# arangesh/TrackMPNN

Hardware: AMD Instinct MI355X
Metric: graph_edges_per_sec_fwd_bwd (higher is better)
Workload: dtype f32; 1 GPU; C2 KITTI Car/RRC-shaped rolling windows: 7 frames, D_t~clip(Poisson(6),1,20), F=8 (2d), H=64, K=0, diff; 1 fwd per frame + 1 bwd per window; 16384 windows/GPU batched block-diagonally (64 distinct seeds tiled); windows_per_gpu=16384, rows_final=6762496, parallelism=sequence-dp1

## Files before the change

include/tmpnn.h:

```cpp
#ifndef TMPNN_H
#define TMPNN_H

#include <stddef.h>
#include <stdint.h>

#ifdef __cplusplus
extern "C" {
#endif

#define TMPNN_ABI_VERSION 10

#define TMPNN_OK 0
#define TMPNN_EINVAL (-1)
#define TMPNN_ELAUNCH (-2)
#define TMPNN_EWORKSPACE (-3)

typedef void* tmpnn_stream;
typedef void* tmpnn_event;

typedef struct tmpnn_seg_plan {
    int32_t T;
    int32_t I;
    int32_t nsplit;
    const int32_t* t_row;
    const int32_t* items;
// ... 99 lines not shown
                          const float* dy, const float* w_head,
                          float* dW_ih, float* dW_hh, float* db_ih, float* db_hh,
                          void* ws, size_t ws_bytes, tmpnn_stream stream);

int tmpnn_gru_bwd_fused_available(int H, int IN, int xmode);
size_t tmpnn_gru_bwd_fused_ws(int R, int IN, int H);
int tmpnn_gru_bwd_fused(const int32_t* rows, int R, int xmode, const int32_t* src, const int32_t* dst,
                        const float* msg, int ld_msg, int msg_compact, int IN,
                        const float* h, int ld_h, int H, const float* w_ih, const float* w_hh,
                        const float* gates, size_t gate_plane, const float* d_hout, int ld_dhout,
                        const float* dy, const float* w_head,
                        float* d_msg, int ld_dmsg, float* d_h, int ld_dh,
                        const int32_t* add_src, const int32_t* add_dst, const float* add_msg, int ld_add,
                        float* dW_ih, float* dW_hh, float* db_ih, float* db_hh,
                        void* ws, size_t ws_bytes, tmpnn_stream stream);
typedef struct tmpnn_zs_gate_src {
    const float* proj;
    int32_t ld_proj;
    const int32_t* src_pos;
    const int32_t* dst_pos;
    const float* b_ih;
    const float* b_hh;
} tmpnn_zs_gate_src;
int tmpnn_gru_bwd_fused_zero_state_available(int H, int IN, int xmode);
int tmpnn_gru_bwd_fused_zero_state(const int32_t* rows, int R, const int32_t* src, const int32_t* dst, int IN,
                                   const float* h, int ld_h, int H, const float* w_ih, const float* b_hn,
                                   const float* gates, size_t gate_plane, const float* d_hout, int ld_dhout,
                                   const float* dy, const float* w_head, float* d_msg, int ld_dmsg,
                                   float* dW_ih, float* db_ih, float* db_hh,
                                   void* ws, size_t ws_bytes, tmpnn_stream stream);

int tmpnn_gru_fwd_tiles(const tmpnn_edge_tiles* tiles, int R, const float* proj, int ld_proj, const float* h, int ld_h, int H,
                        const float* whh_t, const float* b_ih, const float* b_hh, float* h_out, int ld_out, float* gates,
                        size_t gate_plane, const float* w_head, float* logit_part, size_t part_stride, tmpnn_stream stream);
int tmpnn_gru_fwd_tiles_zero_state_available(int H, int xmode);
int tmpnn_gru_fwd_tiles_zero_state(const tmpnn_edge_tiles* tiles, int R, const float* proj, int ld_proj, int H,
                                   const float* b_ih, const float* b_hh, float* h_out, int ld_out, float* gates,
// ... 373 lines not shown
```

trackmpnn_amd/_lib.py:

```python
from __future__ import annotations

import ctypes as C

import torch
import os
import re
from typing import Dict, List, Optional

_HERE = os.path.dirname(os.path.abspath(__file__))
LIB_PATH = os.environ.get('TMPNN_LIB_PATH') or os.path.join(_HERE, 'lib', 'libtmpnn.so')
HEADER_PATH = os.path.join(os.path.dirname(_HERE), 'include', 'tmpnn.h')

ABI_VERSION = 10

c_int = C.c_int
c_void_p = C.c_void_p
c_size_t = C.c_size_t
c_float = C.c_float


class CSegPlan(C.Structure):
    _fields_ = [('T', C.c_int32), ('I', C.c_int32), ('nsplit', C.c_int32), ('t_row', c_void_p), ('items', c_void_p),
                ('rowptr2', c_void_p), ('inc2', c_void_p), ('ws', c_void_p), ('ws_floats', c_size_t)]


class CWinPlan(C.Structure):
    _fields_ = [('W', C.c_int32), ('nbig', C.c_int32), ('wrec', c_void_p), ('erow', c_void_p), ('recs', c_void_p),
                ('det', c_void_p), ('drow', c_void_p), ('big_order', c_void_p)]


class CGraph(C.Structure):
    _fields_ = [('N', C.c_int32), ('E', C.c_int32), ('Dn', C.c_int32),
                ('src', c_void_p), ('dst', c_void_p), ('edge_row', c_void_p), ('det_row', c_void_p),
                ('rowptr', c_void_p), ('inc', c_void_p), ('det_order', c_void_p), ('seg_plan', c_void_p),
                ('win_plan', c_void_p)]


_GP = C.POINTER(CGraph)


class CZsGateSrc(C.Structure):
    _fields_ = [('proj', c_void_p), ('ld_proj', C.c_int32), ('src_pos', c_void_p), ('dst_pos', c_void_p),
                ('b_ih', c_void_p), ('b_hh', c_void_p)]


class CEdgeTiles(C.Structure):
    _fields_ = [('T', C.c_int32), ('rows_per_tile', C.c_int32), ('t_row', c_void_p), ('t_loc', c_void_p),
                ('t_dptr', c_void_p), ('t_dets', c_void_p)]


_TP = C.POINTER(CEdgeTiles)


class CDGraph(C.Structure):
    _fields_ = [('N', C.c_int32), ('cap', C.c_int32), ('meta', c_void_p), ('is_edge', c_void_p), ('pos', c_void_p),
                ('src', c_void_p), ('dst', c_void_p), ('src_pos', c_void_p), ('dst_pos', c_void_p),
                ('edge_row', c_void_p), ('det_row', c_void_p), ('rowptr', c_void_p), ('inc', c_void_p)]

# ... 296 lines not shown
```

trackmpnn_amd/csrc/gru_bwd.hip:

```cpp
#include "gru_common.h"

namespace tmpnn {



template <int NT>
__global__ __launch_bounds__(256) void k_gru_bwd_data(GruBwdDataArgs a) {
    const int wave = threadIdx.x >> 6, lane = threadIdx.x & 63;
    const int c = lane & 31, half = lane >> 5;
    const int r0 = (blockIdx.x * 4 + wave) * 32;
    if (r0 >= a.R) return;
    const int H = a.H;
    const int vcol0 = blockIdx.y * (32 * NT);
    const bool is_dx = vcol0 < a.IN;
    const int n0 = is_dx ? vcol0 : vcol0 - a.IN;
    const float* __restrict__ W = is_dx ? a.w_ih : a.w_hh;
    const int ldw = is_dx ? a.IN : H;
    const int li = min(r0 + c, a.R - 1);
    const int row = a.rows[li];
    const size_t gp = a.gate_plane;

    f32x16 acc[NT];
#pragma unroll
    for (int t = 0; t < NT; ++t)
// ... 1760 lines not shown
        for (int j = 0; j < 3; ++j) {
            const float tot = bsum[j] + __shfl_xor(bsum[j], 32);
            if (half == 0) red[wave * 96 + j * 32 + c32] = tot;
        }
        __syncthreads();
        if (HHS && tt == 0 && half == 0) {
            float* sb = a.slab_b + (size_t)blockIdx.x * 6 * H;
#pragma unroll
            for (int j = 0; j < 3; ++j)
                sb[role * 3 * H + (jt0 + j) * 32 + c32] = red[wave * 96 + j * 32 + c32] + red[(wave + 1) * 96 + j * 32 + c32];
        }
    }
}

struct ZsGateSrc { const float* proj; int ld_proj; const int32_t* src_pos; const int32_t* dst_pos; const float* b_ih; const float* b_hh; };

__device__ __forceinline__ float zs_gate(float ps, float pd, float bsum) { return sigmoidf_((0.0f + (ps - pd)) + bsum); }
__device__ __forceinline__ float zs_gate_n(float ps, float pd, float b_in, float r, float b_hn) {
    return tanhf_(gru_n_preact((ps - pd) + b_in, r, 0.0f + b_hn));
}

template <int UP, bool RC = false>
__global__ __launch_bounds__(512) void k_gru_bwd_zs(GruBwdFusedArgs a, const float* __restrict__ b_hn, int ntiles) {
    constexpr int H = 64;
    constexpr int SUB = 32 * 128;
    constexpr int PA = 2 * SUB, PB = SUB;
    constexpr int OFF_B = 3 * PA;
    constexpr int BUF = OFF_B + 3 * PB;
    extern __shared__ float lds[];
    uint16_t* const lds16 = reinterpret_cast<uint16_t*>(lds);
    const int tid = threadIdx.x;
    const int wave = __builtin_amdgcn_readfirstlane(tid >> 6), lane = tid & 63;
    const int role = wave >> 2, q = wave & 3;
    const int j16 = lane & 15, kq = lane >> 4;
    const int srow = 4 * wave + kq, f4 = 4 * j16;
    const int n0 = 16 * q;
    uint4 wq[6][3];
#pragma unroll
    for (int s6 = 0; s6 < 6; ++s6) {
        const int ch = s6 < 4 ? 4 * kq + s6 : 16 + 4 * (s6 - 4) + kq;
        float v[8];
#pragma unroll
        for (int i = 0; i < 8; ++i) v[i] = a.w_ih[(size_t)(8 * ch + i) * a.ld_wih + n0 + j16];
        const Split8 sp = split8_arr(v);
        wq[s6][0] = sp.p1; wq[s6][1] = sp.p2; wq[s6][2] = sp.p3;
    }
    const float headl = (UP & 2) ? a.up.w_head[lane] : 0.f;
    const float4 bhn = *reinterpret_cast<const float4*>(b_hn + f4);
    const int st0 = dui_off(srow, f4);
    const int swzj = dui_swz(j16), rowj = (16 * role + j16) * 128;
    const int half = lane >> 5, c32 = lane & 31;
    const int jt0 = (q >> 1) * 3, tt = q & 1;
    const int i16 = lane & 15, tq = i16 >> 2, tp = i16 & 3, tg = (lane >> 4) & 1;
    const int trow = (8 * half + tq) * 128, tsw0 = (tq << 2) | (2 * half);
    const int kofs = role * 2048;
    int offA[3], offB;
#pragma unroll
    for (int j = 0; j < 3; ++j) {
        const int col = (jt0 + j) * 32;
        const int ch = ((col & 127) >> 3) + 2 * tg + (tp >> 1);
        offA[j] = kofs + (col >> 7) * SUB + trow + ((ch ^ tsw0) << 3) + 4 * (tp & 1);
    }
    {
// ... 3 lines not shown
    f32x16 acc[3];
#pragma unroll
    for (int j = 0; j < 3; ++j)
#pragma unroll
        for (int i = 0; i < 16; ++i) acc[j][i] = 0.f;
    float bs_r[4] = {0.f, 0.f, 0.f, 0.f}, bs_z[4] = {0.f, 0.f, 0.f, 0.f};
    float bs_n[4] = {0.f, 0.f, 0.f, 0.f}, bs_nr[4] = {0.f, 0.f, 0.f, 0.f};

    const int G = gridDim.x;
    const int nmine = (ntiles - (int)blockIdx.x + G - 1) / G;
    struct { float4 dh, r, z, n, xa, xb; float dy; } raw;
    float d0[4], tv[4];
    struct { float4 pa, pb, qa, qb, na, nb; } rp;
    const ZsGateSrc gsrc{a.msg, a.ld_msg, a.add_src, a.add_dst, a.add_msg, b_hn - 2 * H};
    float* const sgb = lds + BUF;
    if constexpr (RC) {
        if (tid < 3 * H) sgb[tid] = tid < 2 * H ? gsrc.b_ih[tid] + gsrc.b_hh[tid] : gsrc.b_ih[tid];
        __syncthreads();
    }
    auto row_of = [&](int tile, bool tvld, bool& vld) -> int {
        const int lr = tile * 32 + srow;
        vld = tvld && lr < a.R;
        return vld ? lr : a.R - 1;
    };
#define ZS_SLICE(SL, img, vld)                                                                               \
    do {                                                                                                     \
        float o_[4];                                                                                         \
        if ((SL) == 0) {                                                                                     \
            const float dh_[4] = {raw.dh.x, raw.dh.y, raw.dh.z, raw.dh.w}, r_[4] = {raw.r.x, raw.r.y, raw.r.z, raw.r.w}; \
            const float z_[4] = {raw.z.x, raw.z.y, raw.z.z, raw.z.w}, n_[4] = {raw.n.x, raw.n.y, raw.n.z, raw.n.w}; \
            const float hn_[4] = {bhn.x, bhn.y, bhn.z, bhn.w};                                               \
            _Pragma("unroll") for (int i = 0; i < 4; ++i) {                                                  \
// ... 33 lines not shown
            raw.n = TWO_LD4(g0_ + 2 * gp_);                                                                  \
            raw.z = TWO_LD4(g0_ + gp_);                                                                      \
        }                                                                                                    \
    } while (0)
#define ZS_ISSUE_GATHER(gs_, gd_)                                                                            \
    do {                                                                                                     \
        raw.xa = *reinterpret_cast<const float4*>(a.h + (size_t)(gs_) * a.ld_h + f4);                        \
        raw.xb = *reinterpret_cast<const float4*>(a.h + (size_t)(gd_) * a.ld_h + f4);                        \
    } while (0)

#define ZS_ISSUE_P(G3, A_, B_, sp_, dp_)                                                                     \
    do {                                                                                                     \
        rp.A_ = *reinterpret_cast<const float4*>(gsrc.proj + (size_t)(sp_) * gsrc.ld_proj + (G3) * H + f4); \
        rp.B_ = *reinterpret_cast<const float4*>(gsrc.proj + (size_t)(dp_) * gsrc.ld_proj + (G3) * H + f4); \
    } while (0)
#define ZS_GATE(G3, A_, B_, OUT_)                                                                            \
    do {                                                                                                     \
        const float4 b_ = *reinterpret_cast<const float4*>(sgb + (G3) * H + f4);                             \
        raw.OUT_ = make_float4(zs_gate(rp.A_.x, rp.B_.x, b_.x), zs_gate(rp.A_.y, rp.B_.y, b_.y),             \
                               zs_gate(rp.A_.z, rp.B_.z, b_.z), zs_gate(rp.A_.w, rp.B_.w, b_.w));            \
    } while (0)
#define ZS_GATE_N()                                                                                          \
    do {                                                                                                     \
        const float4 b_ = *reinterpret_cast<const float4*>(sgb + 2 * H + f4);                                \
        raw.n = make_float4(zs_gate_n(rp.na.x, rp.nb.x, b_.x, raw.r.x, bhn.x),                               \
                            zs_gate_n(rp.na.y, rp.nb.y, b_.y, raw.r.y, bhn.y),                               \
                            zs_gate_n(rp.na.z, rp.nb.z, b_.z, raw.r.z, bhn.z),                               \
                            zs_gate_n(rp.na.w, rp.nb.w, b_.w, raw.r.w, bhn.w));                              \
    } while (0)
#define ZS_ISSUE_DH(orow_)                                                                                   \
// ... 8 lines not shown
    int sp_n = 0, dp_n = 0;
    if constexpr (RC) {
        bool v0, v1;
        const int lp0 = row_of(blockIdx.x, true, v0);
        const int o0 = a.rows[lp0];
        gs_cur = a.src[lp0]; gd_cur = a.dst[lp0];
        const int sp0 = gsrc.src_pos[lp0], dp0 = gsrc.dst_pos[lp0];
        ZS_ISSUE_DH(o0); ZS_ISSUE_GATHER(gs_cur, gd_cur);
        ZS_ISSUE_P(0, pa, pb, sp0, dp0); ZS_ISSUE_P(1, qa, qb, sp0, dp0); ZS_ISSUE_P(2, na, nb, sp0, dp0);
        const int lp1 = row_of(blockIdx.x + G, 1 < nmine, v1);
        const int o1 = a.rows[lp1];
        const int sp1 = gsrc.src_pos[lp1], dp1 = gsrc.dst_pos[lp1];
        ZS_GATE(0, pa, pb, r); ZS_GATE(1, qa, qb, z); ZS_GATE_N();
        ZS_SLICE(0, lds16, v0); ZS_SLICE(1, lds16, v0); ZS_SLICE(3, lds16, v0); ZS_SLICE(5, lds16, v0);
        ZS_ISSUE_DH(o1);
        ZS_ISSUE_P(0, pa, pb, sp1, dp1); ZS_GATE(0, pa, pb, r);
        ZS_ISSUE_P(1, qa, qb, sp1, dp1); ZS_GATE(1, qa, qb, z);
        ZS_ISSUE_P(2, na, nb, sp1, dp1); ZS_GATE_N();
        valid_cur = v1;
        gs_cur = a.src[lp1]; gd_cur = a.dst[lp1];
        const int lp2 = row_of(blockIdx.x + 2 * G, 2 < nmine, valid_n);
        orow_n = a.rows[lp2];
        sp_n = gsrc.src_pos[lp2]; dp_n = gsrc.dst_pos[lp2];
    } else {
        bool v0, v1;
        const int lp0 = row_of(blockIdx.x, true, v0);
        const int o0 = a.rows[lp0];
        gs_cur = a.src[lp0]; gd_cur = a.dst[lp0];
        ZS_ISSUE_MAIN(0, o0); ZS_ISSUE_MAIN(1, o0); ZS_ISSUE_GATHER(gs_cur, gd_cur);
        const int lp1 = row_of(blockIdx.x + G, 1 < nmine, v1);
        const int o1 = a.rows[lp1];
        ZS_SLICE(0, lds16, v0); ZS_ISSUE_MAIN(0, o1);
        ZS_SLICE(1, lds16, v0); ZS_ISSUE_MAIN(1, o1);
        ZS_SLICE(3, lds16, v0);
        ZS_SLICE(5, lds16, v0);
        valid_cur = v1;
        gs_cur = a.src[lp1]; gd_cur = a.dst[lp1];
        const int lp2 = row_of(blockIdx.x + 2 * G, 2 < nmine, valid_n);
        orow_n = a.rows[lp2];
    }
    __syncthreads();

    for (int it = 0; it < nmine; ++it) {
        const int tile = blockIdx.x + it * G;
        uint16_t* const cur = lds16 + (it & 1) * BUF;
        uint16_t* const nxt = lds16 + ((it & 1) ^ 1) * BUF;
        const int er = a.rows[min(tile * 32 + 16 * role + j16, a.R - 1)];
        const bool el = tile * 32 + 16 * role + j16 < a.R;
        f32x4 accd;
#pragma unroll
        for (int i = 0; i < 4; ++i) accd[i] = 0.f;
#pragma unroll
        for (int s6 = 0; s6 < 6; ++s6) {
            uint4 bd[3];
            const uint16_t* pd;
            {
                const int chunk = s6 < 4 ? 4 * kq + s6 : 4 * (s6 - 4) + kq;
                pd = cur + (s6 >= 4 ? SUB : 0) + rowj + ((chunk ^ swzj) << 3);
            }
            if (s6 < 3) {
                uint4 aw[3], bt[3];
                {
                    const uint16_t* p0 = cur + offB;
                    const uint16_t* p1 = cur + (offB ^ 8) + 4 * 128;
#pragma unroll
                    for (int pc = 0; pc < 3; ++pc) {
                        const uint2 u0 = lds_read_tr(p0 + pc * PB), u1 = lds_read_tr(p1 + pc * PB);
                        bt[pc] = make_uint4(u0.x, u0.y, u1.x, u1.y);
                    }
                }
                const uint16_t* p0 = cur + offA[s6];
                const uint16_t* p1 = cur + (offA[s6] ^ 8) + 4 * 128;
#pragma unroll
                for (int pc = 0; pc < 3; ++pc) {
                    const uint2 u0 = lds_read_tr(p0 + pc * PA), u1 = lds_read_tr(p1 + pc * PA);
                    aw[pc] = make_uint4(u0.x, u0.y, u1.x, u1.y);
                }
                if constexpr (RC) {
                    if (s6 == 0) {
                        ZS_SLICE(0, nxt, valid_cur); ZS_SLICE(1, nxt, valid_cur);
                        ZS_ISSUE_DH(orow_n);
                    } else if (s6 == 1) {
                        ZS_SLICE(3, nxt, valid_cur);
                        ZS_ISSUE_GATHER(gs_cur, gd_cur);
                    } else {
                        ZS_ISSUE_P(0, pa, pb, sp_n, dp_n);
                    }
                } else {
                    ZS_SLICE(s6, nxt, valid_cur);
                    ZS_ISSUE_MAIN(s6, orow_n);
                }
                acc[s6] = mfma32_c<0>(aw, bt, acc[s6]); acc[s6] = mfma32_c<1>(aw, bt, acc[s6]);
                acc[s6] = mfma32_c<2>(aw, bt, acc[s6]); acc[s6] = mfma32_c<3>(aw, bt, acc[s6]);
                acc[s6] = mfma32_c<4>(aw, bt, acc[s6]); acc[s6] = mfma32_c<5>(aw, bt, acc[s6]);
            } else if constexpr (RC) {
                if (s6 == 3) {
                    ZS_SLICE(5, nxt, valid_cur);
                    ZS_ISSUE_P(1, qa, qb, sp_n, dp_n);
                } else if (s6 == 4) {
                    ZS_ISSUE_P(2, na, nb, sp_n, dp_n);
                    ZS_GATE(0, pa, pb, r);
                } else {
                    ZS_GATE(1, qa, qb, z);
                    ZS_GATE_N();
                }
            } else {
                ZS_SLICE(s6, nxt, valid_cur);
                if (s6 == 3) ZS_ISSUE_GATHER(gs_cur, gd_cur);
            }
#pragma unroll
            for (int pc = 0; pc < 3; ++pc) bd[pc] = *reinterpret_cast<const uint4*>(pd + pc * PA);
            accd = mfma16_c<0>(wq[s6], bd, accd); accd = mfma16_c<1>(wq[s6], bd, accd);
            accd = mfma16_c<2>(wq[s6], bd, accd); accd = mfma16_c<3>(wq[s6], bd, accd);
            accd = mfma16_c<4>(wq[s6], bd, accd); accd = mfma16_c<5>(wq[s6], bd, accd);
            __builtin_amdgcn_sched_barrier(0);
        }
        {
            bool vnn;
            const int lp2 = row_of(tile + 2 * G, it + 2 < nmine, vnn);
            gs_cur = a.src[lp2]; gd_cur = a.dst[lp2];
            valid_cur = valid_n;
            const int lp3 = row_of(tile + 3 * G, it + 3 < nmine, valid_n);
            orow_n = a.rows[lp3];
            if constexpr (RC) { sp_n = gsrc.src_pos[lp3]; dp_n = gsrc.dst_pos[lp3]; }
            (void)vnn;
        }
        int cofs = n0 + 4 * kq;
        asm volatile("" : "+v"(cofs));
        if (el) *reinterpret_cast<float4*>(a.d_msg + ((size_t)er * a.ld_dmsg + cofs)) =
                    make_float4(accd[0], accd[1], accd[2], accd[3]);
        __syncthreads();
    }
#undef ZS_ISSUE_DH
#undef ZS_GATE_N
#undef ZS_GATE
#undef ZS_ISSUE_P
#undef ZS_ISSUE_GATHER
#undef ZS_ISSUE_MAIN
#undef ZS_SLICE
    float* sw = a.slab_w + (size_t)blockIdx.x * (3 * H) * (2 * H);
#pragma unroll
    for (int j = 0; j < 3; ++j)
#pragma unroll
        for (int reg = 0; reg < 16; ++reg) {
            const int jj = (jt0 + j) * 32 + acc_row(reg, half);
            sw[(size_t)jj * (2 * H) + role * H + tt * 32 + c32] = acc[j][reg];
        }
    {
        float* red = lds;
        *reinterpret_cast<float4*>(red + srow * 256 + 0 * 64 + f4) = make_float4(bs_r[0], bs_r[1], bs_r[2], bs_r[3]);
// ... 380 lines not shown
int tmpnn_gru_bwd_fused_zero_state_available(int H, int IN, int xmode) {
    return (H == 64 && IN == 64 && xmode == 1 && device_gives_160k()) ? 1 : 0;
}

int tmpnn_gru_bwd_fused_zero_state(const int32_t* rows, int R, const int32_t* src, const int32_t* dst, int IN,
                                   const float* h, int ld_h, int H, const float* w_ih, const float* b_hn,
                                   const float* gates, size_t gate_plane, const float* d_hout, int ld_dhout,
                                   const float* dy, const float* w_head, float* d_msg, int ld_dmsg, float* dW_ih,
                                   float* db_ih, float* db_hh, void* ws, size_t ws_bytes, tmpnn_stream stream) {
    TM_REQUIRE(tmpnn_gru_bwd_fused_zero_state_available(H, IN, 1), "gru_bwd_fused_zero_state: H=%d IN=%d not supported", H, IN);
    if (R == 0) return TMPNN_OK;
    TM_REQUIRE(R > 0 && rows && src && dst && h && w_ih && b_hn && gates && d_msg && dW_ih && db_ih && db_hh,
               "gru_bwd_fused_zero_state: null pointer");
    const bool rc_gates = gate_plane == 0;
    ZsGateSrc gsrc{};
    if (rc_gates) {
        const tmpnn_zs_gate_src* g = reinterpret_cast<const tmpnn_zs_gate_src*>(gates);
        TM_REQUIRE(g->proj && g->src_pos && g->dst_pos && g->b_ih && g->b_hh,
                   "gru_bwd_fused_zero_state: gate_plane = 0 needs proj, src_pos, dst_pos, b_ih and b_hh (struct tmpnn_zs_gate_src)");
        TM_REQUIRE(aligned16(g->proj) && g->ld_proj >= 3 * H && (g->ld_proj & 3) == 0 && aligned16(g->b_ih) && aligned16(g->b_hh),
                   "gru_bwd_fused_zero_state: gate source layout (16-byte alignment, ld_proj=%d)", (int)g->ld_proj);
        TM_REQUIRE(b_hn == g->b_hh + 2 * H, "gru_bwd_fused_zero_state: b_hn is not b_hh + 2H of the gate source");
        gsrc = ZsGateSrc{g->proj, g->ld_proj, g->src_pos, g->dst_pos, g->b_ih, g->b_hh};
        gates = nullptr;
    }
    TM_REQUIRE(d_hout != nullptr || dy != nullptr, "gru_bwd_fused_zero_state: no upstream gradient");
    TM_REQUIRE(dy == nullptr || (w_head != nullptr && aligned16(w_head)),
               "gru_bwd_fused_zero_state: dy needs a 16-byte aligned w_head");
    TM_REQUIRE((ld_h & 3) == 0 && aligned16(h) && aligned16(gates) && (gate_plane & 3) == 0 && aligned16(w_ih) &&
                   aligned16(b_hn) && (d_hout == nullptr || ((ld_dhout & 3) == 0 && aligned16(d_hout))) &&
                   (ld_dmsg & 3) == 0 && aligned16(d_msg) && ld_dmsg >= IN && ld_h >= H,
               "gru_bwd_fused_zero_state: rows must be 16-byte aligned");
    const size_t need = tmpnn_gru_bwd_fused_ws(R, IN, H);
    if (ws == nullptr || ws_bytes < need)
        return set_error(TMPNN_EWORKSPACE, "gru_bwd_fused_zero_state: workspace %zu < %zu bytes", ws_bytes, need);
    const int n_rs = fused_blocks(R);
    const size_t nW = (size_t)3 * H * (IN + H), nB = (size_t)6 * H;
    float* slab_w = reinterpret_cast<float*>(ws);
    float* slab_b = slab_w + (size_t)n_rs * nW;
    float* fold = slab_b + (size_t)n_rs * nB;
    GruBwdFusedArgs a{rows, R, src, dst, nullptr, 0, 0, h, ld_h, w_ih, nullptr, gates, gate_plane,
                      DhSrc{d_hout, ld_dhout, dy, w_head}, d_msg, ld_dmsg, nullptr, 0, nullptr, nullptr, nullptr, 0,
                      slab_w, slab_b, IN};
    if (rc_gates) {
        a.msg = gsrc.proj; a.ld_msg = gsrc.ld_proj;
        a.add_src = gsrc.src_pos; a.add_dst = gsrc.dst_pos; a.add_msg = gsrc.b_ih;
    }
    const int ntiles = ceil_div(R, 32);
    const size_t shm = 147456;
    hipStream_t st = as_stream(stream);
    const int up = (d_hout ? 1 : 0) | (dy ? 2 : 0);
#define LZ(U)                                                                                                \
    do {                                                                                                     \
        TM_SHM_ONCE((k_gru_bwd_zs<U>), shm);                                                                 \
        hipLaunchKernelGGL((k_gru_bwd_zs<U>), dim3(n_rs), dim3(512), shm, st, a, b_hn, ntiles);              \
    } while (0)
#define LZR(U)                                                                                               \
    do {                                                                                                     \
        TM_SHM_ONCE((k_gru_bwd_zs<U, true>), shm + 3 * H * sizeof(float));                                   \
        hipLaunchKernelGGL((k_gru_bwd_zs<U, true>), dim3(n_rs), dim3(512), shm + 3 * H * sizeof(float), st, a, b_hn, ntiles); \
    } while (0)
    if (rc_gates) {
        if (up == 1) LZR(1); else if (up == 2) LZR(2); else LZR(3);
    } else {
        if (up == 1) LZ(1); else if (up == 2) LZ(2); else LZ(3);
    }
#undef LZR
#undef LZ
    int rc = check_launch("gru_bwd_fused_zero_state");
    if (rc) return rc;
    const float* rw = slab_w;
    const float* rb = slab_b;
    int nred = n_rs;
    if (n_rs > 64) {
        const int ng = ceil_div(n_rs, 32);
        float* fw = fold;
        float* fb = fold + (size_t)ng * nW;
        hipLaunchKernelGGL(k_fold_slabs_gru, dim3(ceil_div((long)nW, 256), ng), dim3(256), 0, st, slab_w, nW, n_rs, fw, nW);
        hipLaunchKernelGGL(k_fold_slabs_gru, dim3(ceil_div((long)nB, 256), ng), dim3(256), 0, st, slab_b, nB, n_rs, fb, nB);
        if ((rc = check_launch("gru_fold"))) return rc;
        rw = fw; rb = fb; nred = ng;
// ... 137 lines not shown
```

trackmpnn_amd/functional.py:

```python
from __future__ import annotations

import contextlib
import ctypes
import os
from dataclasses import dataclass
from typing import Dict, List, Optional, Sequence, Tuple

import torch

from . import _lib
from .graph import CallPlan, dense_seg_plan, edge_tiles, win_plan

ATT_DROPOUT_P = 0.5
INPLACE_GRADS = os.environ.get('TMPNN_INPLACE_GRADS', '0') == '1'
FUSED_BWD = os.environ.get('TMPNN_FUSED_BWD', '1') == '1'
ZERO_STATE_BWD = os.environ.get('TMPNN_BWD_ZERO_STATE', '1') != '0'
ZERO_STATE_FWD = os.environ.get('TMPNN_FWD_ZERO_STATE', '1') != '0'
WIDE_OVERLAP = os.environ.get('TMPNN_WIDE_OVERLAP', '0') == '1' and os.environ.get('TMPNN_KEEP_VARIANTS', '0') == '1'
ATT_KMAX = 8
_SPLIT = os.environ.get('TMPNN_SPLIT', '1')[:1] != '0'

_VARIANTS = os.environ.get('TMPNN_KEEP_VARIANTS', '0') == '1'


def _variant(name: str, default: str) -> str:
    return os.environ.get(name, default) if _VARIANTS else default


WIDE_DW = _variant('TMPNN_WIDE_DW', '1') == '1'
WIDE_DET = _variant('TMPNN_WIDE_DET', '1') == '1'
WIDE = _variant('TMPNN_WIDE', '1') != '0' and _SPLIT
WIDE_TILED = _variant('TMPNN_WIDE_TILED', '1') != '0'
FWD_TILED = _variant('TMPNN_FWD_TILED', '1') != '0' and _SPLIT
FWD_TILE_ROWS = 16 if _variant('TMPNN_FWD_TILE_ROWS', '32') == '16' else 32
INPUT_TF = _variant('TMPNN_INPUT_TF', '1') != '0'
RECOMPUTE_GATES = _variant('TMPNN_RECOMPUTE_GATES', '0') == '1'
CONCAT_PROJ = _variant('TMPNN_CONCAT_PROJ', '1') != '0'
ZS_RECOMPUTE = _variant('TMPNN_ZS_RECOMPUTE', '1') != '0'
WIN_SEGSUM = _variant('TMPNN_SEGSUM_WIN', '0') == '1'
WIDE_FUSED_ADJOINT = _variant('TMPNN_WIDE_FUSED_ADJOINT', '1') != '0'
_aux_streams: Dict[torch.device, 'torch.cuda.Stream'] = {}


def _aux_stream(dev) -> Optional[int]:
    if not WIDE_OVERLAP or torch.cuda.is_current_stream_capturing():
        return None
    key = torch.device(dev)
    s = _aux_streams.get(key)
    if s is None:
        s = torch.cuda.Stream(key)
        _aux_streams[key] = s
    if s.cuda_stream == torch.cuda.current_stream(key).cuda_stream:
        return None
# ... 327 lines not shown
            if FWD_TILED and E > 0:
                recompute = RECOMPUTE_GATES and save
                E_full = E_old if zs_fwd else E
                if E_full > 0:
                    tiles = edge_tiles(g, FWD_TILE_ROWS, e1=E_full)
                    _lib.call('tmpnn_gru_fwd_tiles', tiles.cref(), E_full, proj.data_ptr(), 3 * H, hg, GH, H,
                              e_whh_t.data_ptr(), P[f + 'edge_gru.bias_ih'].data_ptr(), P[f + 'edge_gru.bias_hh'].data_ptr(),
                              og, GH, None if recompute else gp, plane, we_g, part_g, N, st)
                if zs_fwd:
                    _lib.call('tmpnn_gru_fwd_tiles_zero_state', edge_tiles(g, FWD_TILE_ROWS, e0=E_old).cref(), E - E_old,
                              proj.data_ptr(), 3 * H, H, P[f + 'edge_gru.bias_ih'].data_ptr(),
                              P[f + 'edge_gru.bias_hh'].data_ptr(), og, GH, None if zs_rc else gp, plane,
                              int(save and not zs_bwd), we_g, part_g, N, st)
                    if zs_rc:
                        saved['zs_rc']['proj'][gi] = proj
                if recompute:
                    saved.setdefault('proj', {})[gi] = (proj, e_whh_t)
            else:
                _lib.call('tmpnn_gru_fwd', g.edge_row.data_ptr(), E, 3, g.src_pos.data_ptr(), g.dst_pos.data_ptr(),
                          proj.data_ptr(), 3 * H, 0, H, hg, GH, H, None, e_whh_t.data_ptr(),
                          P[f + 'edge_gru.bias_ih'].data_ptr(), P[f + 'edge_gru.bias_hh'].data_ptr(),
                          og, GH, gp, plane, we_g, part_g, N, st)
        else:
            _lib.call('tmpnn_gru_fwd', g.edge_row.data_ptr(), E, xmode, g.src.data_ptr(), g.dst.data_ptr(),
                      None, 0, 0, spec.IN_e, hg, GH, H,
                      e_wih_t.data_ptr(), e_whh_t.data_ptr(),
                      P[f + 'edge_gru.bias_ih'].data_ptr(), P[f + 'edge_gru.bias_hh'].data_ptr(),
                      og, GH, gp, plane, we_g, part_g, N, st)
        es = es_all[gi]
        if K == 0:
# ... 153 lines not shown
                          None, 0, 0, IN_e, hg, GH, H,
                          P[f + 'edge_gru.weight_ih'].data_ptr(), P[f + 'edge_gru.weight_hh'].data_ptr(),
                          gp, plane, dog, GH, dyp, we, dmsg.data_ptr(), IN_e, dhg, GH,
                          g.src.data_ptr() if fuse else None, g.dst.data_ptr() if fuse else None,
                          dmsg.data_ptr() if fuse else None, IN_e,
                          grads[f + 'edge_gru.weight_ih'].data_ptr(), grads[f + 'edge_gru.weight_hh'].data_ptr(),
                          grads[f + 'edge_gru.bias_ih'].data_ptr(), grads[f + 'edge_gru.bias_hh'].data_ptr(),
                          ws_w.data_ptr(), ws_w.numel() * 4, st)
            if zs:
                zg, zplane = gp, plane
                rc = saved.get('zs_rc')
                if rc is not None:
                    src_ = _lib.CZsGateSrc(rc['proj'][gi].data_ptr(), 3 * H, rc['src_pos'].data_ptr() + 4 * E_old,
                                           rc['dst_pos'].data_ptr() + 4 * E_old, P[f + 'edge_gru.bias_ih'].data_ptr(),
                                           P[f + 'edge_gru.bias_hh'].data_ptr())
                    zg, zplane = ctypes.addressof(src_), 0
                _lib.call('tmpnn_gru_bwd_fused_zero_state', g.edge_row.data_ptr() + 4 * E_old, E - E_old,
                          g.src.data_ptr() + 4 * E_old, g.dst.data_ptr() + 4 * E_old, IN_e, hg, GH, H,
                          P[f + 'edge_gru.weight_ih'].data_ptr(), b_hn, zg, zplane, dog, GH, dyp, we,
                          dmsg.data_ptr(), IN_e, grads[f + 'edge_gru.weight_ih'].data_ptr(),
                          grads[f + 'edge_gru.bias_ih'].data_ptr(), grads[f + 'edge_gru.bias_hh'].data_ptr(),
                          ws_w.data_ptr(), ws_w.numel() * 4, st)
        else:
            _lib.call('tmpnn_gru_bwd_data', g.det_row.data_ptr(), Dn, H, hg, GH, H,
                      P[f + 'node_gru.weight_ih'].data_ptr(), P[f + 'node_gru.weight_hh'].data_ptr(),
                      gp, plane, dog, GH, dyp, wn, dmsg.data_ptr(), IN_e, dhg, GH, None, None, None, 0, st)
            _lib.call('tmpnn_gru_bwd_weights', g.det_row.data_ptr(), Dn, 0, None, None, es.data_ptr(), H, 1, H,
                      hg, GH, H, gp, plane, dog, GH, dyp, wn,
                      grads[f + 'node_gru.weight_ih'].data_ptr(), grads[f + 'node_gru.weight_hh'].data_ptr(),
                      grads[f + 'node_gru.bias_ih'].data_ptr(), grads[f + 'node_gru.bias_hh'].data_ptr(),
# ... 188 lines not shown
```

trackmpnn_amd/graph.py:

```python
from __future__ import annotations

import ctypes as C
from dataclasses import dataclass, field
from typing import List, Optional, Sequence, Tuple

import numpy as np
import torch

from . import _lib


@dataclass
class FrameGraph:
    N: int
    E: int
    Dn: int
    src: torch.Tensor
    dst: torch.Tensor
    edge_row: torch.Tensor
    det_row: torch.Tensor
    rowptr: torch.Tensor
    inc: torch.Tensor
    is_edge: torch.Tensor
    pos: torch.Tensor
# ... 60 lines not shown
        endpoint = (self.inc < 0).long()
        epos = torch.full((self.N,), -1, dtype=torch.long, device=self.device)
        epos[self.edge_row.long()] = torch.arange(self.E, device=self.device)
        return epos[row], endpoint


@dataclass
class EdgeTiles:
    T: int
    rows_per_tile: int
    t_row: torch.Tensor
    t_loc: torch.Tensor
    t_dptr: torch.Tensor
    t_dets: torch.Tensor
    max_dets: int = 0
    _c: Optional[_lib.CEdgeTiles] = field(default=None, repr=False, compare=False)

    def cref(self):
        if self._c is None:
            self._c = _lib.CEdgeTiles(self.T, self.rows_per_tile, self.t_row.data_ptr(), self.t_loc.data_ptr(),
                                      self.t_dptr.data_ptr(), self.t_dets.data_ptr())
        return C.byref(self._c)


def build_edge_tiles(graph: FrameGraph, rows_per_tile: int = 128, src_group: int = 8, dst_group: int = 16,
                     stats: bool = False, order: str = 'blocks', dst_offset: int = 0,
                     e0: int = 0, e1: Optional[int] = None) -> EdgeTiles:
    if graph.src_pos is None or graph.dst_pos is None:
        raise ValueError('build_edge_tiles: the graph carries no src_pos / dst_pos')
    dev = graph.device
    e1 = graph.E if e1 is None else int(e1)
    e0 = int(e0)
    if not 0 <= e0 <= e1 <= graph.E:
        raise ValueError(f'build_edge_tiles: edge range [{e0}, {e1}) outside [0, {graph.E})')
    E, R = e1 - e0, int(rows_per_tile)
    T = (E + R - 1) // R
    i32 = lambda t: t.to(torch.int32).contiguous()
    if T == 0:
        z = torch.zeros(0, dtype=torch.int32, device=dev)
        return EdgeTiles(0, R, z, z.clone(), torch.zeros(1, dtype=torch.int32, device=dev), z.clone())
    s, d = graph.src_pos[e0:e1].long(), graph.dst_pos[e0:e1].long()
    ns = graph.Dn // src_group + 1
    if order == 'rows':
        so, do, ro = s, d, graph.edge_row[e0:e1].long()
    else:
        key = (((d // dst_group) * ns + s // src_group) * src_group + s % src_group) * dst_group + d % dst_group
        perm = torch.argsort(key)
        so, do, ro = s[perm], d[perm], graph.edge_row[e0:e1].long()[perm]
    pad = T * R - E
    if pad:
        so = torch.cat([so, so[-1:].expand(pad)])
        do = torch.cat([do, do[-1:].expand(pad)])
        ro = torch.cat([ro, torch.full((pad,), -1, dtype=torch.long, device=dev)])
    both = torch.cat([so.view(T, R), do.view(T, R) + int(dst_offset)], 1)
    vals, perm = both.sort(1)
    first = torch.ones_like(vals, dtype=torch.bool)
    first[:, 1:] = vals[:, 1:] != vals[:, :-1]
    rank = first.long().cumsum(1) - 1
    local = torch.empty_like(rank)
    local.scatter_(1, perm, rank)
    cnt = rank[:, -1] + 1
    dptr = torch.zeros(T + 1, dtype=torch.long, device=dev)
    dptr[1:] = cnt.cumsum(0)
    loc = local[:, :R] | (local[:, R:] << 16)
    tiles = EdgeTiles(T, R, i32(ro), i32(loc.reshape(-1)), i32(dptr), i32(vals[first]))
    if stats:
        tiles.max_dets = int(cnt.max())
    return tiles


def edge_tiles(graph: FrameGraph, rows_per_tile: int = 128, dst_offset: int = 0, e0: int = 0,
               e1: Optional[int] = None) -> EdgeTiles:
    cache = graph.__dict__.setdefault('_tiles', {})
    e1 = graph.E if e1 is None else int(e1)
    key = rows_per_tile if not dst_offset else (rows_per_tile, int(dst_offset))
    if (int(e0), e1) != (0, graph.E):
        key = (key, int(e0), e1)
    t = cache.get(key)
    if t is None:
        runs = 1
# ... 1 lines not shown
            if graph.src_pos.is_cuda and torch.cuda.is_current_stream_capturing():
                raise RuntimeError('edge_tiles: the tile list of this graph is not built yet and building it reads one '
                                   'count back to the host, which a stream capture cannot do -- run one eager call on the '
                                   'graph (CapturedWindow does) before capturing')
            runs = 1 + int((graph.src_pos[1:] != graph.src_pos[:-1]).sum())
        blocks = graph.E / runs >= rows_per_tile / 2
        od = 'blocks' if blocks else 'rows'
        rng = dict(order=od, dst_offset=dst_offset, e0=e0, e1=e1)
        if rows_per_tile == 128:
            t = build_edge_tiles(graph, 128, 8, 16, **rng)
        elif rows_per_tile == 16:
            t = build_edge_tiles(graph, 16, 4, 4, **rng)
        else:
            t = build_edge_tiles(graph, rows_per_tile, 4, 8, **rng)
        cache[key] = t
    return t


class SegPlan:

    def __init__(self, T, I, nsplit, t_row, items, rowptr2, inc2, ws):
        self.T, self.I, self.nsplit = int(T), int(I), int(nsplit)
        self.t_row, self.items, self.rowptr2, self.inc2, self.ws = t_row, items, rowptr2, inc2, ws
        self.c = _lib.CSegPlan(self.T, self.I, self.nsplit, t_row.data_ptr(), items.data_ptr(), rowptr2.data_ptr(),
                               inc2.data_ptr(), ws.data_ptr(), ws.numel())


SEG_ITEM_TILES = 13


# ... 649 lines not shown
```

Before: 746.3 million graph-edges/s.

## Stage per-tile detection projections in LDS for zero-state GRU backward recompute

Adds a tile-staged variant of the zero-state fused GRU backward kernel. It loads each 32-row tile's distinct detection projection rows into LDS once, through the edge-tile list (t_loc/t_dptr/t_dets), and reads the src/dst gate operands from LDS. Previously every edge gathered those operands from global memory. The change also threads a tiles pointer through the ABI and builds row-ordered tile lists in the forward pass. The cost is more LDS, extra scalar loads and pipeline complexity, and a fallback to global gathers when a tile has more than 32 distinct detections.

```diff
diff --git a/include/tmpnn.h b/include/tmpnn.h
--- a/include/tmpnn.h
+++ b/include/tmpnn.h
@@ -8,7 +8,7 @@
 extern "C" {
 #endif
 
-#define TMPNN_ABI_VERSION 10
+#define TMPNN_ABI_VERSION 11
 
 #define TMPNN_OK 0
 #define TMPNN_EINVAL (-1)
@@ -138,6 +138,7 @@
                         const int32_t* add_src, const int32_t* add_dst, const float* add_msg, int ld_add,
                         float* dW_ih, float* dW_hh, float* db_ih, float* db_hh,
                         void* ws, size_t ws_bytes, tmpnn_stream stream);
+#define TMPNN_ZS_STAGE_MAX_DETS 32
 typedef struct tmpnn_zs_gate_src {
     const float* proj;
     int32_t ld_proj;
@@ -145,6 +146,7 @@
     const int32_t* dst_pos;
     const float* b_ih;
     const float* b_hh;
+    const tmpnn_edge_tiles* tiles;
 } tmpnn_zs_gate_src;
 int tmpnn_gru_bwd_fused_zero_state_available(int H, int IN, int xmode);
 int tmpnn_gru_bwd_fused_zero_state(const int32_t* rows, int R, const int32_t* src, const int32_t* dst, int IN,
diff --git a/trackmpnn_amd/_lib.py b/trackmpnn_amd/_lib.py
--- a/trackmpnn_amd/_lib.py
+++ b/trackmpnn_amd/_lib.py
@@ -11,7 +11,7 @@
 LIB_PATH = os.environ.get('TMPNN_LIB_PATH') or os.path.join(_HERE, 'lib', 'libtmpnn.so')
 HEADER_PATH = os.path.join(os.path.dirname(_HERE), 'include', 'tmpnn.h')
 
-ABI_VERSION = 10
+ABI_VERSION = 11
 
 c_int = C.c_int
 c_void_p = C.c_void_p
@@ -41,7 +41,7 @@
 
 class CZsGateSrc(C.Structure):
     _fields_ = [('proj', c_void_p), ('ld_proj', C.c_int32), ('src_pos', c_void_p), ('dst_pos', c_void_p),
-                ('b_ih', c_void_p), ('b_hh', c_void_p)]
+                ('b_ih', c_void_p), ('b_hh', c_void_p), ('tiles', c_void_p)]
 
 
 class CEdgeTiles(C.Structure):
diff --git a/trackmpnn_amd/csrc/gru_bwd.hip b/trackmpnn_amd/csrc/gru_bwd.hip
--- a/trackmpnn_amd/csrc/gru_bwd.hip
+++ b/trackmpnn_amd/csrc/gru_bwd.hip
@@ -1798,13 +1798,14 @@
 }
 
 struct ZsGateSrc { const float* proj; int ld_proj; const int32_t* src_pos; const int32_t* dst_pos; const float* b_ih; const float* b_hh; };
+constexpr int ZS_STAGE_CAP = 32;
 
 __device__ __forceinline__ float zs_gate(float ps, float pd, float bsum) { return sigmoidf_((0.0f + (ps - pd)) + bsum); }
 __device__ __forceinline__ float zs_gate_n(float ps, float pd, float b_in, float r, float b_hn) {
     return tanhf_(gru_n_preact((ps - pd) + b_in, r, 0.0f + b_hn));
 }
 
-template <int UP, bool RC = false>
+template <int UP, bool RC = false, bool TS = false>
 __global__ __launch_bounds__(512) void k_gru_bwd_zs(GruBwdFusedArgs a, const float* __restrict__ b_hn, int ntiles) {
     constexpr int H = 64;
     constexpr int SUB = 32 * 128;
@@ -1830,7 +1831,8 @@
         wq[s6][0] = sp.p1; wq[s6][1] = sp.p2; wq[s6][2] = sp.p3;
     }
     const float headl = (UP & 2) ? a.up.w_head[lane] : 0.f;
-    const float4 bhn = *reinterpret_cast<const float4*>(b_hn + f4);
+    const float4 bhn_r = *reinterpret_cast<const float4*>(b_hn + (TS ? 0 : f4));
+#define bhn (TS ? *reinterpret_cast<const float4*>(lds + BUF + 3 * H + f4) : bhn_r)
     const int st0 = dui_off(srow, f4);
     const int swzj = dui_swz(j16), rowj = (16 * role + j16) * 128;
     const int half = lane >> 5, c32 = lane & 31;
@@ -1864,8 +1866,21 @@
     struct { float4 pa, pb, qa, qb, na, nb; } rp;
     const ZsGateSrc gsrc{a.msg, a.ld_msg, a.add_src, a.add_dst, a.add_msg, b_hn - 2 * H};
     float* const sgb = lds + BUF;
+    static_assert(!TS || RC, "the tile stage belongs to the recompute form");
+    auto stage_off = [&](int p, int g, int f4_) -> int {
+        const int u = 3 * p + g, piece = u >> 4, rp2 = u & 15;
+        const int base16 = piece < 3 ? OFF_B + piece * PB : (piece - 3) * PA + SUB;
+        return (base16 >> 1) + (2 * rp2 + (f4_ >> 5)) * 64 + ((rp2 & 1) ? 0 : 32) + (f4_ & 31);
+    };
+    const int32_t* const tl_loc = reinterpret_cast<const int32_t*>(a.w_hh);
+    typedef const int32_t __attribute__((address_space(4))) zs_cint;
+    zs_cint* const tl_dptr_c = (zs_cint*)reinterpret_cast<const int32_t*>(a.gates);
+    const int32_t* const tl_dets = reinterpret_cast<const int32_t*>(a.d_h);
+    int loc_rd = 0, db_rd = 0, n_rd = 0, fdet = 0, db_f = 0, n_f = 0, dq0 = 0, dq1 = 0;
+    auto tile_c = [&](int t) -> int { return min(t, ntiles - 1); };
     if constexpr (RC) {
         if (tid < 3 * H) sgb[tid] = tid < 2 * H ? gsrc.b_ih[tid] + gsrc.b_hh[tid] : gsrc.b_ih[tid];
+        if (TS && tid < H) sgb[3 * H + tid] = b_hn[tid];
         __syncthreads();
     }
     auto row_of = [&](int tile, bool tvld, bool& vld) -> int {
@@ -1929,6 +1944,16 @@
         rp.A_ = *reinterpret_cast<const float4*>(gsrc.proj + (size_t)(sp_) * gsrc.ld_proj + (G3) * H + f4); \
         rp.B_ = *reinterpret_cast<const float4*>(gsrc.proj + (size_t)(dp_) * gsrc.ld_proj + (G3) * H + f4); \
     } while (0)
+#define ZS_LDS_P(G3, A_, B_)                                                                                 \
+    do {                                                                                                     \
+        const float* nf_ = reinterpret_cast<const float*>(nxt);                                              \
+        int l_ = loc_rd, f_ = f4;                                                                            \
+        asm volatile("" : "+v"(l_), "+v"(f_));              \
+        rp.A_ = *reinterpret_cast<const float4*>(nf_ + stage_off(min(l_ & 0xffff, ZS_STAGE_CAP - 1), (G3), f_)); \
+        rp.B_ = *reinterpret_cast<const float4*>(nf_ + stage_off(min((int)((unsigned)l_ >> 16), ZS_STAGE_CAP - 1), (G3), f_)); \
+    } while (0)
+#define ZS_FILL() (n_f <= ZS_STAGE_CAP && srow < n_f)
+#define ZS_FDET() (ZS_FILL() ? tl_dets[db_f + srow] : 0)
 #define ZS_GATE(G3, A_, B_, OUT_)                                                                            \
     do {                                                                                                     \
         const float4 b_ = *reinterpret_cast<const float4*>(sgb + (G3) * H + f4);                             \
@@ -1967,14 +1992,34 @@
         ZS_GATE(0, pa, pb, r); ZS_GATE(1, qa, qb, z); ZS_GATE_N();
         ZS_SLICE(0, lds16, v0); ZS_SLICE(1, lds16, v0); ZS_SLICE(3, lds16, v0); ZS_SLICE(5, lds16, v0);
         ZS_ISSUE_DH(o1);
-        ZS_ISSUE_P(0, pa, pb, sp1, dp1); ZS_GATE(0, pa, pb, r);
-        ZS_ISSUE_P(1, qa, qb, sp1, dp1); ZS_GATE(1, qa, qb, z);
-        ZS_ISSUE_P(2, na, nb, sp1, dp1); ZS_GATE_N();
+        if constexpr (!TS) {
+            ZS_ISSUE_P(0, pa, pb, sp1, dp1); ZS_GATE(0, pa, pb, r);
+            ZS_ISSUE_P(1, qa, qb, sp1, dp1); ZS_GATE(1, qa, qb, z);
+            ZS_ISSUE_P(2, na, nb, sp1, dp1); ZS_GATE_N();
+        }
         valid_cur = v1;
         gs_cur = a.src[lp1]; gd_cur = a.dst[lp1];
         const int lp2 = row_of(blockIdx.x + 2 * G, 2 < nmine, valid_n);
         orow_n = a.rows[lp2];
-        sp_n = gsrc.src_pos[lp2]; dp_n = gsrc.dst_pos[lp2];
+        if constexpr (TS) {
+            const int t1 = tile_c(blockIdx.x + G), t2 = tile_c(blockIdx.x + 2 * G), t3 = tile_c(blockIdx.x + 3 * G);
+            db_rd = __builtin_amdgcn_readfirstlane(tl_dptr_c[t1]);
+            n_rd = __builtin_amdgcn_readfirstlane(tl_dptr_c[t1 + 1]) - db_rd;
+            loc_rd = tl_loc[t1 * 32 + srow];
+            if (n_rd <= ZS_STAGE_CAP && srow < n_rd) {
+                const float* fp = gsrc.proj + (size_t)tl_dets[db_rd + srow] * gsrc.ld_proj + f4;
+#pragma unroll
+                for (int g3 = 0; g3 < 3; ++g3)
+                    *reinterpret_cast<float4*>(lds + (BUF >> 1) + stage_off(srow, g3, f4)) = *reinterpret_cast<const float4*>(fp + g3 * H);
+            }
+            db_f = __builtin_amdgcn_readfirstlane(tl_dptr_c[t2]);
+            n_f = __builtin_amdgcn_readfirstlane(tl_dptr_c[t2 + 1]) - db_f;
+            fdet = ZS_FDET();
+            dq0 = __builtin_amdgcn_readfirstlane(tl_dptr_c[t3]);
+            dq1 = __builtin_amdgcn_readfirstlane(tl_dptr_c[t3 + 1]);
+        } else {
+            sp_n = gsrc.src_pos[lp2]; dp_n = gsrc.dst_pos[lp2];
+        }
     } else {
         bool v0, v1;
         const int lp0 = row_of(blockIdx.x, true, v0);
@@ -2003,6 +2048,9 @@
         f32x4 accd;
 #pragma unroll
         for (int i = 0; i < 4; ++i) accd[i] = 0.f;
+        float4 fq0, fq1, fq2;
+        const bool fill = TS && ZS_FILL();
+        const bool st_rd = TS && n_rd <= ZS_STAGE_CAP;
 #pragma unroll
         for (int s6 = 0; s6 < 6; ++s6) {
             uint4 bd[3];
@@ -2029,7 +2077,25 @@
                     const uint2 u0 = lds_read_tr(p0 + pc * PA), u1 = lds_read_tr(p1 + pc * PA);
                     aw[pc] = make_uint4(u0.x, u0.y, u1.x, u1.y);
                 }
-                if constexpr (RC) {
+                if constexpr (TS) {
+                    if (s6 == 0) {
+                        if (fill) {
+                            const float* fp = gsrc.proj + (size_t)fdet * gsrc.ld_proj + f4;
+                            fq0 = *reinterpret_cast<const float4*>(fp); fq1 = *reinterpret_cast<const float4*>(fp + H);
+                            fq2 = *reinterpret_cast<const float4*>(fp + 2 * H);
+                        }
+                    } else if (s6 == 2) {
+                        if (fill) {
+                            float* cf_ = reinterpret_cast<float*>(cur);
+                            int sr_ = srow, f_ = f4;
+                            asm volatile("" : "+v"(sr_), "+v"(f_));
+                            *reinterpret_cast<float4*>(cf_ + stage_off(sr_, 0, f_)) = fq0;
+                            *reinterpret_cast<float4*>(cf_ + stage_off(sr_, 1, f_)) = fq1;
+                            *reinterpret_cast<float4*>(cf_ + stage_off(sr_, 2, f_)) = fq2;
+                        }
+                        ZS_ISSUE_GATHER(gs_cur, gd_cur);
+                    }
+                } else if constexpr (RC) {
                     if (s6 == 0) {
                         ZS_SLICE(0, nxt, valid_cur); ZS_SLICE(1, nxt, valid_cur);
                         ZS_ISSUE_DH(orow_n);
@@ -2046,6 +2112,23 @@
                 acc[s6] = mfma32_c<0>(aw, bt, acc[s6]); acc[s6] = mfma32_c<1>(aw, bt, acc[s6]);
                 acc[s6] = mfma32_c<2>(aw, bt, acc[s6]); acc[s6] = mfma32_c<3>(aw, bt, acc[s6]);
                 acc[s6] = mfma32_c<4>(aw, bt, acc[s6]); acc[s6] = mfma32_c<5>(aw, bt, acc[s6]);
+            } else if constexpr (TS) {
+                if (s6 == 3) {
+                    if (st_rd) {
+                        ZS_LDS_P(0, pa, pb); ZS_LDS_P(1, qa, qb);
+                    } else {
+                        sp_n = tl_dets[db_rd + (loc_rd & 0xffff)]; dp_n = tl_dets[db_rd + (int)((unsigned)loc_rd >> 16)];
+                        ZS_ISSUE_P(0, pa, pb, sp_n, dp_n); ZS_ISSUE_P(1, qa, qb, sp_n, dp_n);
+                    }
+                    ZS_GATE(0, pa, pb, r); ZS_GATE(1, qa, qb, z);
+                } else if (s6 == 4) {
+                    if (st_rd) ZS_LDS_P(2, na, nb); else ZS_ISSUE_P(2, na, nb, sp_n, dp_n);
+                    ZS_GATE_N();
+                    ZS_SLICE(0, nxt, valid_cur); ZS_SLICE(1, nxt, valid_cur); ZS_SLICE(3, nxt, valid_cur);
+                    ZS_ISSUE_DH(orow_n);
+                } else {
+                    ZS_SLICE(5, nxt, valid_cur);
+                }
             } else if constexpr (RC) {
                 if (s6 == 3) {
                     ZS_SLICE(5, nxt, valid_cur);
@@ -2075,7 +2158,15 @@
             valid_cur = valid_n;
             const int lp3 = row_of(tile + 3 * G, it + 3 < nmine, valid_n);
             orow_n = a.rows[lp3];
-            if constexpr (RC) { sp_n = gsrc.src_pos[lp3]; dp_n = gsrc.dst_pos[lp3]; }
+            if constexpr (TS) {
+                loc_rd = tl_loc[tile_c(tile + 2 * G) * 32 + srow];
+                db_rd = db_f; n_rd = n_f;
+                db_f = dq0; n_f = dq1 - dq0;
+                fdet = ZS_FDET();
+                const int t4 = tile_c(tile + 4 * G);
+                dq0 = __builtin_amdgcn_readfirstlane(tl_dptr_c[t4]);
+                dq1 = __builtin_amdgcn_readfirstlane(tl_dptr_c[t4 + 1]);
+            } else if constexpr (RC) { sp_n = gsrc.src_pos[lp3]; dp_n = gsrc.dst_pos[lp3]; }
             (void)vnn;
         }
         int cofs = n0 + 4 * kq;
@@ -2087,6 +2178,10 @@
 #undef ZS_ISSUE_DH
 #undef ZS_GATE_N
 #undef ZS_GATE
+#undef ZS_LDS_P
+#undef ZS_FILL
+#undef ZS_FDET
+#undef bhn
 #undef ZS_ISSUE_P
 #undef ZS_ISSUE_GATHER
 #undef ZS_ISSUE_MAIN
@@ -2497,6 +2592,7 @@
                "gru_bwd_fused_zero_state: null pointer");
     const bool rc_gates = gate_plane == 0;
     ZsGateSrc gsrc{};
+    const tmpnn_edge_tiles* tl = nullptr;
     if (rc_gates) {
         const tmpnn_zs_gate_src* g = reinterpret_cast<const tmpnn_zs_gate_src*>(gates);
         TM_REQUIRE(g->proj && g->src_pos && g->dst_pos && g->b_ih && g->b_hh,
@@ -2505,6 +2601,18 @@
                    "gru_bwd_fused_zero_state: gate source layout (16-byte alignment, ld_proj=%d)", (int)g->ld_proj);
         TM_REQUIRE(b_hn == g->b_hh + 2 * H, "gru_bwd_fused_zero_state: b_hn is not b_hh + 2H of the gate source");
         gsrc = ZsGateSrc{g->proj, g->ld_proj, g->src_pos, g->dst_pos, g->b_ih, g->b_hh};
+        if (g->tiles) {
+            TM_REQUIRE((reinterpret_cast<uintptr_t>(g->tiles) & (alignof(tmpnn_edge_tiles) - 1)) == 0,
+                       "gru_bwd_fused_zero_state: misaligned tiles");
+            tl = g->tiles;
+            TM_REQUIRE(tl->rows_per_tile == 32 && tl->T == ceil_div(R, 32),
+                       "gru_bwd_fused_zero_state: tiles (T=%d, rows_per_tile=%d) is not the list of these %d rows in 32-row tiles",
+                       (int)tl->T, (int)tl->rows_per_tile, R);
+            TM_REQUIRE(tl->t_loc && tl->t_dptr && tl->t_dets &&
+                           ((reinterpret_cast<uintptr_t>(tl->t_loc) | reinterpret_cast<uintptr_t>(tl->t_dptr) |
+                             reinterpret_cast<uintptr_t>(tl->t_dets)) & 3) == 0,
+                       "gru_bwd_fused_zero_state: tiles needs 4-byte aligned t_loc, t_dptr and t_dets");
+        }
         gates = nullptr;
     }
     TM_REQUIRE(d_hout != nullptr || dy != nullptr, "gru_bwd_fused_zero_state: no upstream gradient");
@@ -2528,6 +2636,11 @@
     if (rc_gates) {
         a.msg = gsrc.proj; a.ld_msg = gsrc.ld_proj;
         a.add_src = gsrc.src_pos; a.add_dst = gsrc.dst_pos; a.add_msg = gsrc.b_ih;
+        if (tl) {
+            a.w_hh = reinterpret_cast<const float*>(tl->t_loc);
+            a.gates = reinterpret_cast<const float*>(tl->t_dptr);
+            a.d_h = reinterpret_cast<float*>(const_cast<int32_t*>(tl->t_dets));
+        }
     }
     const int ntiles = ceil_div(R, 32);
     const size_t shm = 147456;
@@ -2543,11 +2656,19 @@
         TM_SHM_ONCE((k_gru_bwd_zs<U, true>), shm + 3 * H * sizeof(float));                                   \
         hipLaunchKernelGGL((k_gru_bwd_zs<U, true>), dim3(n_rs), dim3(512), shm + 3 * H * sizeof(float), st, a, b_hn, ntiles); \
     } while (0)
-    if (rc_gates) {
+#define LZT(U)                                                                                               \
+    do {                                                                                                     \
+        TM_SHM_ONCE((k_gru_bwd_zs<U, true, true>), shm + 4 * H * sizeof(float));                             \
+        hipLaunchKernelGGL((k_gru_bwd_zs<U, true, true>), dim3(n_rs), dim3(512), shm + 4 * H * sizeof(float), st, a, b_hn, ntiles); \
+    } while (0)
+    if (rc_gates && tl) {
+        if (up == 1) LZT(1); else if (up == 2) LZT(2); else LZT(3);
+    } else if (rc_gates) {
         if (up == 1) LZR(1); else if (up == 2) LZR(2); else LZR(3);
     } else {
         if (up == 1) LZ(1); else if (up == 2) LZ(2); else LZ(3);
     }
+#undef LZT
 #undef LZR
 #undef LZ
     int rc = check_launch("gru_bwd_fused_zero_state");
diff --git a/trackmpnn_amd/functional.py b/trackmpnn_amd/functional.py
--- a/trackmpnn_amd/functional.py
+++ b/trackmpnn_amd/functional.py
@@ -9,7 +9,7 @@
 import torch
 
 from . import _lib
-from .graph import CallPlan, dense_seg_plan, edge_tiles, win_plan
+from .graph import CallPlan, dense_seg_plan, edge_tiles, edge_tiles_in_order, win_plan
 
 ATT_DROPOUT_P = 0.5
 INPLACE_GRADS = os.environ.get('TMPNN_INPLACE_GRADS', '0') == '1'
@@ -37,6 +37,8 @@
 RECOMPUTE_GATES = _variant('TMPNN_RECOMPUTE_GATES', '0') == '1'
 CONCAT_PROJ = _variant('TMPNN_CONCAT_PROJ', '1') != '0'
 ZS_RECOMPUTE = _variant('TMPNN_ZS_RECOMPUTE', '1') != '0'
+ZS_TILE_STAGE = _variant('TMPNN_ZS_TILE_STAGE', '1') != '0'
+ZS_STAGE_MAX_DETS = 32
 WIN_SEGSUM = _variant('TMPNN_SEGSUM_WIN', '0') == '1'
 WIDE_FUSED_ADJOINT = _variant('TMPNN_WIDE_FUSED_ADJOINT', '1') != '0'
 _aux_streams: Dict[torch.device, 'torch.cuda.Stream'] = {}
@@ -394,6 +396,8 @@
                               int(save and not zs_bwd), we_g, part_g, N, st)
                     if zs_rc:
                         saved['zs_rc']['proj'][gi] = proj
+                        if ZS_TILE_STAGE and gi == 0:
+                            edge_tiles_in_order(g, FWD_TILE_ROWS, e0=E_old)
                 if recompute:
                     saved.setdefault('proj', {})[gi] = (proj, e_whh_t)
             else:
@@ -577,6 +581,9 @@
                     src_ = _lib.CZsGateSrc(rc['proj'][gi].data_ptr(), 3 * H, rc['src_pos'].data_ptr() + 4 * E_old,
                                            rc['dst_pos'].data_ptr() + 4 * E_old, P[f + 'edge_gru.bias_ih'].data_ptr(),
                                            P[f + 'edge_gru.bias_hh'].data_ptr())
+                    tl = edge_tiles_in_order(g, FWD_TILE_ROWS, e0=E_old, build=False) if ZS_TILE_STAGE else None
+                    if tl is not None and tl.T == (E - E_old + 31) // 32 and tl.rows_per_tile == 32:
+                        src_.tiles = ctypes.cast(tl.cref(), ctypes.c_void_p).value
                     zg, zplane = ctypes.addressof(src_), 0
                 _lib.call('tmpnn_gru_bwd_fused_zero_state', g.edge_row.data_ptr() + 4 * E_old, E - E_old,
                           g.src.data_ptr() + 4 * E_old, g.dst.data_ptr() + 4 * E_old, IN_e, hg, GH, H,
diff --git a/trackmpnn_amd/graph.py b/trackmpnn_amd/graph.py
--- a/trackmpnn_amd/graph.py
+++ b/trackmpnn_amd/graph.py
@@ -98,6 +98,7 @@
     t_dptr: torch.Tensor
     t_dets: torch.Tensor
     max_dets: int = 0
+    order: str = 'blocks'
     _c: Optional[_lib.CEdgeTiles] = field(default=None, repr=False, compare=False)
 
     def cref(self):
@@ -122,7 +123,7 @@
     i32 = lambda t: t.to(torch.int32).contiguous()
     if T == 0:
         z = torch.zeros(0, dtype=torch.int32, device=dev)
-        return EdgeTiles(0, R, z, z.clone(), torch.zeros(1, dtype=torch.int32, device=dev), z.clone())
+        return EdgeTiles(0, R, z, z.clone(), torch.zeros(1, dtype=torch.int32, device=dev), z.clone(), order=order)
     s, d = graph.src_pos[e0:e1].long(), graph.dst_pos[e0:e1].long()
     ns = graph.Dn // src_group + 1
     if order == 'rows':
@@ -147,7 +148,7 @@
     dptr = torch.zeros(T + 1, dtype=torch.long, device=dev)
     dptr[1:] = cnt.cumsum(0)
     loc = local[:, :R] | (local[:, R:] << 16)
-    tiles = EdgeTiles(T, R, i32(ro), i32(loc.reshape(-1)), i32(dptr), i32(vals[first]))
+    tiles = EdgeTiles(T, R, i32(ro), i32(loc.reshape(-1)), i32(dptr), i32(vals[first]), order=order)
     if stats:
         tiles.max_dets = int(cnt.max())
     return tiles
@@ -179,6 +180,24 @@
         else:
             t = build_edge_tiles(graph, rows_per_tile, 4, 8, **rng)
         cache[key] = t
+    return t
+
+
+def edge_tiles_in_order(graph: FrameGraph, rows_per_tile: int = 32, e0: int = 0, e1: Optional[int] = None,
+                        build: bool = True) -> Optional[EdgeTiles]:
+    cache = graph.__dict__.get('_tiles', {}) if not build else graph.__dict__.setdefault('_tiles', {})
+    e1 = graph.E if e1 is None else int(e1)
+    key = rows_per_tile
+    if (int(e0), e1) != (0, graph.E):
+        key = (key, int(e0), e1)
+    t = cache.get(key)
+    if t is not None and t.order == 'rows':
+        return t
+    t = cache.get(('rows', key))
+    if t is None and build:
+        t = edge_tiles(graph, rows_per_tile, e0=e0, e1=e1)
+        if t.order != 'rows':
+            t = cache[('rows', key)] = build_edge_tiles(graph, rows_per_tile, 4, 8, order='rows', e0=e0, e1=e1)
     return t
 
 
```

Result: slower. 725.8 million graph-edges/s (-2.7%).
